# davidlougheed/strkit

Measured on NVIDIA B200. Metric: read x locus repeat counts per second, higher is better.
Workload: dtype u16x2/int32

## Files before the change

strkit_b200/csrc/api.cu:

```cuda
#include <algorithm>
#include <chrono>
#include <cmath>
#include <cstdarg>
#include <cstdio>
#include <cstdlib>
#include <cstring>
#include <mutex>
#include <new>
#include <vector>

#include "../../include/strkit_b200.h"
#include "dp_general.cuh"
#include "dp_packed.cuh"
#include "plan.cuh"
#include "dedupe.cuh"
#include "int_peak.cuh"
#include "replay.cuh"
#include "ref_path.cuh"
#include "strk_common.cuh"

static thread_local char g_err[512] = "";

static int set_err(int code, const char *fmt, ...) {
    va_list ap;
// ... 1525 lines not shown
                    const int fl = lens[3 * l], fr = lens[3 * l + 2], m = motif_len[l];
                    lists.add(strk_pk_class(fl, lens[3 * l + 1], fr, m), (int)l, m, fl, fr);
                }
                if (ctx->fallback.reserve(n) != cudaSuccess) {
                    cudaGetLastError();
                    return set_err(STRK_ERR_NOMEM, "strk_ref_counts: cannot allocate the fallback list");
                }
                const int *seg_list[STRK_PK_NBIN];
                long long seg_cnt[STRK_PK_NBIN];
                int seg_w[STRK_PK_NBIN];
                for (int k = 0; k < STRK_PK_NBIN; ++k) seg_w[k] = 2 * stride_w - 1;
                rc = lists.upload(d.lists, st, seg_list, seg_cnt);
                if (rc) return rc;
                CU(cudaMemsetAsync(ctx->d_queue + 2, 0, sizeof(unsigned int), st));
                long long n_packed = 0;
                rc = launch_pass(ctx, seg_list, seg_cnt, lists.flank, lists.mmax, seg_w, n_loci, ctx->fams.p, d.arena.p,
                                 ctx->table64.p, b_len, rowlen, st, 1, &n_packed);
                if (rc) return rc;
                CU(cudaStreamSynchronize(st));
            } else {
                rc = launch_general(ctx, true, ctx->fams.p, nullptr, n_pending, d.arena.p, ctx->table64.p, b_len, rowlen, st);
                if (rc) return rc;
            }
            CU(cudaEventRecord(ctx->ev[1], st));
            CU(cudaMemsetAsync(d.cnt.p, 0, 4 * sizeof(unsigned int), st));
            ref_replay1_kernel<<<(unsigned)((n_pending + T - 1) / T), T, 0, st>>>(
                d_ids, (int)n_pending, ctx->table64.p, ctx->fams.p, d.start.p, d.rc.p, d.ref_size.p, vcf_anchor_size, WD_MAX,
                d.wd.p, d.l_off.p, d.r_off.p, d.n_off.p, d_again, d.cnt.p);
            CU(cudaGetLastError());
            CU(cudaEventRecord(ctx->ev[2], st));
            ctx->stats[2] += 2;
            unsigned int h_cnt[4] = {0, 0, 0, 0};
            CU(cudaMemcpyAsync(h_cnt, d.cnt.p, sizeof(h_cnt), cudaMemcpyDeviceToHost, st));
            CU(cudaStreamSynchronize(st));
            {
                float t0 = 0.f, t1 = 0.f;
                CU(cudaEventElapsedTime(&t0, ctx->ev[0], ctx->ev[1]));
                CU(cudaEventElapsedTime(&t1, ctx->ev[1], ctx->ev[2]));
                acc_stats[3] += t0;
                acc_stats[4] += t1;
            }
            if (h_cnt[2])
                return set_err(STRK_ERR_SEARCH, "strk_ref_counts: locus %lld left the widest window",
                               (long long)(0x7fffffffu - h_cnt[2]));
            if (h_cnt[1]) {
                const long long l = (long long)(0x7fffffffu - h_cnt[1]);
                return set_err(STRK_ERR_SEARCH, "strk_ref_counts: locus %lld scored no size (max_iters = %d)", l,
                               rc_params[3 * l]);
            }
            n_pending = h_cnt[0];
            acc_stats[5] += (double)n_pending;
            d_ids = d_again;
            d_again = d_again == d.ids_a.p ? d.ids_b.p : d.ids_a.p;
            cur_wd = std::min(WD_MAX, cur_wd * 4);
        }
    }
    const double t_phase1 = now();
    acc_stats[2] = ctx->stats[2];
    std::vector<int> l_off(n), r_off(n), n_off(n);
    CU(cudaMemcpyAsync(l_off.data(), d.l_off.p, n * sizeof(int), cudaMemcpyDeviceToHost, st));
    CU(cudaMemcpyAsync(r_off.data(), d.r_off.p, n * sizeof(int), cudaMemcpyDeviceToHost, st));
    CU(cudaMemcpyAsync(n_off.data(), d.n_off.p, n * sizeof(int), cudaMemcpyDeviceToHost, st));

    std::vector<std::vector<int>> tiers;
    std::vector<int> tier_key;
    for (int64_t l = 0; l < n_loci; ++l) {
        size_t t = 0;
        for (; t < tiers.size(); ++t)
            if (tier_key[3 * t] == rc_params[3 * l] && tier_key[3 * t + 1] == rc_params[3 * l + 1] &&
                tier_key[3 * t + 2] == rc_params[3 * l + 2])
                break;
        if (t == tiers.size()) {
            tiers.emplace_back();
            tier_key.insert(tier_key.end(), rc_params + 3 * l, rc_params + 3 * l + 3);
        }
        tiers[t].push_back((int)l);
    }
    if (!ctx->ref_batch) ctx->ref_batch = new (std::nothrow) strk_batch();
    if (!ctx->ref_batch) return set_err(STRK_ERR_NOMEM, "out of host memory");
    strk_batch *b = ctx->ref_batch;
    std::vector<int> res;
    for (size_t t = 0; t < tiers.size(); ++t) {
        const std::vector<int> &ids = tiers[t];
        const size_t nt = ids.size();
        const cudaError_t e = batch_bind(b, (long long)nt, (long long)nt);
        if (e != cudaSuccess) {
            cudaGetLastError();
            return set_err(STRK_ERR_NOMEM, "strk_ref_counts: %s", cudaGetErrorString(e));
        }
        b->d_arena = d.arena.p;
        b->h_read_begin.resize(nt + 1);
        for (size_t q = 0; q <= nt; ++q) b->h_read_begin[q] = (long long)q;
        CU(cudaMemcpyAsync(d.ids_a.p, ids.data(), nt * sizeof(int), cudaMemcpyHostToDevice, st));
        ref_plan2_kernel<<<(unsigned)((nt + T - 1) / T), T, 0, st>>>(d.ids_a.p, (int)nt, d.seq_off.p, d.lens.p, d.start.p,
                                                                     d.motif_off.p, d.motif_len.p, d.l_off.p, d.r_off.p,
                                                                     b->d_seq_off, b->d_lens, b->d_est, b->d_motif_off,
                                                                     b->d_motif_len, b->d_read_begin);
        CU(cudaGetLastError());
        CU(cudaStreamSynchronize(st));
        rc = batch_plan(ctx, b, arena_bytes);
        if (rc) return rc;
        rc = strk_batch_run(ctx, b, tier_key[3 * t], tier_key[3 * t + 1], tier_key[3 * t + 2], STRK_KERNEL_AUTO, nullptr);
        if (rc) return rc;
        for (int k = 0; k < 8; ++k) acc_stats[k] += ctx->stats[k];
        res.resize(nt * 4);
        CU(cudaMemcpy(res.data(), b->d_out, nt * 4 * sizeof(int), cudaMemcpyDeviceToHost));
        for (size_t q = 0; q < nt; ++q) {
            const int l = ids[q];
            int32_t *o = out + 8 * (size_t)l;
            o[0] = res[4 * q], o[1] = res[4 * q + 1], o[2] = l_off[(size_t)l], o[3] = r_off[(size_t)l];
            o[4] = n_off[(size_t)l], o[5] = res[4 * q + 2];
            o[6] = lens[3 * l] - std::max(0, l_off[(size_t)l]);
            o[7] = lens[3 * l + 2] - std::max(0, r_off[(size_t)l]);
        }
    }
    for (int k = 0; k < 8; ++k) ctx->stats[k] = acc_stats[k];
    if (timing)
        fprintf(stderr, "[strk_ref_counts] %lld loci: upload + phase 1 %.2f ms, phase 2 %.2f ms (host clock); DP kernels %.2f ms, "
                "replay kernels %.2f ms (device clock), %d kernels\n", (long long)n_loci, t_phase1 - t_begin, now() - t_phase1,
                acc_stats[3], acc_stats[4], (int)acc_stats[2]);
    return STRK_OK;
}

static int ref_counts_fast(strk_ctx *ctx, const uint8_t *arena, uint64_t arena_bytes, const uint64_t *seq_off,
                           const int32_t *lens, const int32_t *start_count, const int32_t *ref_size,
                           const int32_t *rc_params, int64_t n_loci, const uint64_t *motif_off, const int32_t *motif_len,
                           int vcf_anchor_size, int32_t *out, std::vector<int> &redo, bool *taken) {
    *taken = false;
    if (!ctx->h_consts.packed_ok) return STRK_OK;
    for (int64_t l = 1; l < n_loci; ++l)
        if (rc_params[3 * l] != rc_params[0] || rc_params[3 * l + 1] != rc_params[1] || rc_params[3 * l + 2] != rc_params[2])
            return STRK_OK;
    const int max_iters = rc_params[0], range = rc_params[1], step = rc_params[2];
    if (max_iters < 0 || range < 0 || step < 0 || range > 1000 || step > 1000)
        return set_err(STRK_ERR_ARG, "strk_ref_counts: bad search parameters");
    const int wd1 = ref_first_wd(range, step);
    const int stride_w = 2 * wd1 + 1;
    int wd2 = range + step + 2;
    if (wd2 < 6) wd2 = 6;
    const int W2 = 2 * wd2 + 1;
    if (2 * stride_w > PK_WINDOW_MAX || W2 > PK_WINDOW_MAX) return STRK_OK;
    *taken = true;
    cudaStream_t st = ctx->stream;
    int rc = ref_setup(ctx, st, arena, arena_bytes, seq_off, lens, start_count, ref_size, rc_params, n_loci, motif_off,
                       motif_len);
    if (rc) return rc;
    RefBufs &d = ctx->ref;
    const size_t n = (size_t)n_loci;
    int max_n1 = 0, mb_cols = 0, mb_m = 0;
    ClassLists &lists = d.classes;
    lists.clear();
    double cells1 = 0.0;
    for (int64_t l = 0; l < n_loci; ++l) {
        const int fl = lens[3 * l], tr = lens[3 * l + 1], fr = lens[3 * l + 2], m = motif_len[l];
        const int n1 = fl + tr + fr;
        max_n1 = std::max(max_n1, n1);
        if (n1 > 32 * 16) {
            mb_cols = std::max(mb_cols, std::max(fl, fr) + m * (start_count[l] + (fl + fr) / m + 1));
            mb_m = std::max(mb_m, m);
        }
        lists.add(strk_pk_class(fl, tr, fr, m), (int)l, m, fl, fr);
        cells1 += (double)n1 * ((double)fl + fr + 2.0 * m * ((double)start_count[l] + wd1));
    }
    if (!ctx->ref_batch) ctx->ref_batch = new (std::nothrow) strk_batch();
    if (!ctx->ref_batch) return set_err(STRK_ERR_NOMEM, "out of host memory");
    strk_batch *b = ctx->ref_batch;
    const int CAP2 = 4096;
    const int WD_MAX = (STRK_MAX_WINDOW - 1) / 2;
    const int wd1b = std::min(WD_MAX, 4 * wd1), stride_w2 = 2 * wd1b + 1;
    cudaError_t e = d.out.reserve(8 * n + 8);
    if (e == cudaSuccess) e = batch_bind(b, (long long)n, (long long)n);
    if (e == cudaSuccess) e = ctx->fams.reserve(std::max(n, (size_t)CAP2));
    if (e == cudaSuccess) e = ctx->table64.reserve(std::max(n * (size_t)stride_w * 2, (size_t)CAP2 * (size_t)stride_w2 * 2));
    if (e == cudaSuccess) e = ctx->table.reserve(n * (size_t)W2);
    if (e == cudaSuccess) e = ctx->fallback.reserve(n);
    if (e != cudaSuccess) {
        cudaGetLastError();
        return set_err(STRK_ERR_NOMEM, "strk_ref_counts: %s", cudaGetErrorString(e));
    }
    b->d_arena = d.arena.p;
    const int *seg_list[STRK_PK_NBIN];
    long long seg_cnt[STRK_PK_NBIN];
    rc = lists.upload(d.lists, st, seg_list, seg_cnt);
    if (rc) return rc;
    CU(cudaMemsetAsync(d.cnt.p, 0, 8 * sizeof(unsigned int), st));
    CU(cudaMemsetAsync(ctx->d_acc, 0, 4 * sizeof(double), st));
    CU(cudaMemsetAsync(ctx->d_queue + 1, 0, 3 * sizeof(unsigned int), st));
    const int T = 128;
    const int b_len = max_n1 + 2;
    const int rowlen = max_n1 > 32 * 16 ? mb_cols + mb_m * std::max(std::max(wd1, wd2), wd1b) + 2 : 2;
    int seg_w1[STRK_PK_NBIN], seg_w2[STRK_PK_NBIN];
    for (int k = 0; k < STRK_PK_NBIN; ++k) {
        seg_w1[k] = 2 * stride_w - 1;
        seg_w2[k] = (W2 + 3) / 4 * 4;
    }
    ref_plan1_kernel<<<(unsigned)((n + T - 1) / T), T, 0, st>>>(nullptr, (int)n, d.seq_off.p, d.lens.p, d.start.p, d.wd.p,
                                                               d.motif_off.p, d.motif_len.p, stride_w, ctx->fams.p);
    CU(cudaGetLastError());
    CU(cudaEventRecord(ctx->ev[0], st));
    long long n_packed = 0;
    rc = launch_pass(ctx, seg_list, seg_cnt, lists.flank, lists.mmax, seg_w1, n_loci, ctx->fams.p, d.arena.p, ctx->table64.p,
                     b_len, rowlen, st, 1, &n_packed);
    if (rc) return rc;
    CU(cudaEventRecord(ctx->ev[1], st));
    ref_replay1_kernel<<<(unsigned)((n + T - 1) / T), T, 0, st>>>(nullptr, (int)n, ctx->table64.p, ctx->fams.p, d.start.p, d.rc.p,
                                                                 d.ref_size.p, vcf_anchor_size, WD_MAX, d.wd.p, d.l_off.p,
                                                                 d.r_off.p, d.n_off.p, d.ids_a.p, d.cnt.p);
    CU(cudaGetLastError());
    {
        ref_clamp_count_kernel<<<1, 32, 0, st>>>(d.cnt.p, (unsigned)CAP2);
        ref_plan1_kernel<<<(unsigned)((CAP2 + T - 1) / T), T, 0, st>>>(d.ids_a.p, CAP2, d.seq_off.p, d.lens.p, d.start.p, d.wd.p,
                                                                      d.motif_off.p, d.motif_len.p, stride_w2, ctx->fams.p, d.cnt.p);
        CU(cudaGetLastError());
        rc = launch_general(ctx, true, ctx->fams.p, nullptr, CAP2, d.arena.p, ctx->table64.p, b_len, rowlen, st, d.cnt.p);
        if (rc) return rc;
        ref_replay1_kernel<<<(unsigned)((CAP2 + T - 1) / T), T, 0, st>>>(d.ids_a.p, CAP2, ctx->table64.p, ctx->fams.p, d.start.p,
                                                                        d.rc.p, d.ref_size.p, vcf_anchor_size, WD_MAX, d.wd.p,
                                                                        d.l_off.p, d.r_off.p, d.n_off.p, d.ids_b.p, d.cnt.p + 4,
                                                                        d.cnt.p);
        CU(cudaGetLastError());
    }
    ref_plan2_kernel<<<(unsigned)((n + T - 1) / T), T, 0, st>>>(nullptr, (int)n, d.seq_off.p, d.lens.p, d.start.p, d.motif_off.p,
                                                               d.motif_len.p, d.l_off.p, d.r_off.p, b->d_seq_off, b->d_lens,
                                                               b->d_est, b->d_motif_off, b->d_motif_len, b->d_read_begin,
                                                               b->d_read_locus);
    CU(cudaGetLastError());
    plan_reads_kernel<<<(unsigned)((n + 255) / 256), 256, 0, st>>>(nullptr, (long long)n, b->d_seq_off, b->d_lens, b->d_est,
                                                                  b->d_read_locus, b->d_motif_off, b->d_motif_len, wd2, 0, W2,
                                                                  ctx->fams.p, ctx->d_acc + 1, nullptr);
    CU(cudaGetLastError());
    CU(cudaEventRecord(ctx->ev[2], st));
    CU(cudaMemsetAsync(ctx->d_queue + 2, 0, sizeof(unsigned int), st));
    long long n_packed2 = 0;
    rc = launch_pass(ctx, seg_list, seg_cnt, lists.flank, lists.mmax, seg_w2, n_loci, ctx->fams.p, d.arena.p, ctx->table.p, b_len,
                     rowlen, st, 0, &n_packed2);
    if (rc) return rc;
    CU(cudaEventRecord(ctx->ev[3], st));
    rc = launch_replay(ctx, b, W2, wd2, 0, nullptr, nullptr, (long long)n, max_iters, range, step, nullptr, nullptr, st);
    if (rc) return rc;
    ref_assemble_kernel<<<(unsigned)((n + T - 1) / T), T, 0, st>>>((int)n, b->d_out, b->d_status, d.lens.p, d.l_off.p, d.r_off.p,
                                                                  d.n_off.p, d.out.p);
    CU(cudaGetLastError());
    CU(cudaEventRecord(ctx->ev[4], st));
    std::vector<unsigned char> status(n);
    unsigned int h_cnt[8] = {0, 0, 0, 0, 0, 0, 0, 0};
    double acc[2] = {0, 0};
    CU(cudaMemcpyAsync(out, d.out.p, 8 * n * sizeof(int), cudaMemcpyDeviceToHost, st));
    CU(cudaMemcpyAsync(status.data(), b->d_status, n, cudaMemcpyDeviceToHost, st));
    CU(cudaMemcpyAsync(h_cnt, d.cnt.p, sizeof(h_cnt), cudaMemcpyDeviceToHost, st));
    CU(cudaMemcpyAsync(acc, ctx->d_acc, sizeof(acc), cudaMemcpyDeviceToHost, st));
    CU(cudaStreamSynchronize(st));
    if (h_cnt[1] || h_cnt[5]) {
        const long long l = (long long)(0x7fffffffu - (h_cnt[1] ? h_cnt[1] : h_cnt[5]));
        return set_err(STRK_ERR_SEARCH, "strk_ref_counts: locus %lld scored no size (max_iters = %d)", l, max_iters);
    }
    for (size_t l = 0; l < n; ++l)
        if (status[l] || out[8 * l + 4] < 0) redo.push_back((int)l);
    float t1 = 0.f, t2 = 0.f, t3 = 0.f, t4 = 0.f;
    CU(cudaEventElapsedTime(&t1, ctx->ev[0], ctx->ev[1]));
    CU(cudaEventElapsedTime(&t2, ctx->ev[1], ctx->ev[2]));
    CU(cudaEventElapsedTime(&t3, ctx->ev[2], ctx->ev[3]));
    CU(cudaEventElapsedTime(&t4, ctx->ev[3], ctx->ev[4]));
    ctx->stats[0] = cells1 + acc[1];
    ctx->stats[1] = acc[0];
    ctx->stats[2] += 7;
    ctx->stats[3] = t1 + t3;
    ctx->stats[4] = t2 + t4;
    ctx->stats[5] = 0;
    if (getenv("STRK_REF_TIMING"))
        fprintf(stderr, "[strk_ref_counts] fast path, %lld loci: DP kernels %.2f + %.2f ms, replay / second look / planning kernels "
                "%.2f + %.2f ms (device clock), %u loci took the second look, %zu left to redo\n", (long long)n_loci, t1, t3, t2, t4,
                h_cnt[0], redo.size());
    return STRK_OK;
}

extern "C" int strk_measure_int_peak(strk_ctx *ctx, double out_tiops[3]) {
    if (!ctx || !out_tiops) return set_err(STRK_ERR_ARG, "strk_measure_int_peak: null argument");
    CU(cudaSetDevice(ctx->device));
    int *d_out = (int *)(ctx->d_queue + 7);
    const int grid = ctx->n_sm * 8, threads = 256, iters = 4096;
    const double instr = (double)grid * threads * (double)iters * 64.0;
    cudaEvent_t e0 = ctx->ev[0], e1 = ctx->ev[1];
    for (int mode = 0; mode < 3; ++mode) {
        float best = 1e30f;
        for (int rep = 0; rep < 4; ++rep) {
            CU(cudaEventRecord(e0, ctx->stream));
            if (mode == 0) int_peak_kernel<0><<<grid, threads, 0, ctx->stream>>>(iters, rep + 3, d_out);
            if (mode == 1) int_peak_kernel<1><<<grid, threads, 0, ctx->stream>>>(iters, rep + 3, d_out);
            if (mode == 2) int_peak_kernel<2><<<grid, threads, 0, ctx->stream>>>(iters, rep + 3, d_out);
            CU(cudaGetLastError());
            CU(cudaEventRecord(e1, ctx->stream));
            CU(cudaEventSynchronize(e1));
            float ms = 0.f;
            CU(cudaEventElapsedTime(&ms, e0, e1));
            if (rep > 0 && ms < best) best = ms;
        }
        out_tiops[mode] = instr / ((double)best * 1e-3) / 1e12;
    }
    return STRK_OK;
}

#include "alleles_api.cuh"
#include "realign_api.cuh"
```

strkit_b200/csrc/dp_packed.cuh:

```cuda
#pragma once
#include "dp_general.cuh"
#include "strk_common.cuh"

#define PK_FLANK_MAX 160
#define PK_WINDOW_MAX 128
#ifndef PK_WARPS
#define PK_WARPS 4
#endif
#ifndef PK_WARPS_PAIRED
#define PK_WARPS_PAIRED 4
#endif
__host__ __device__ constexpr int pk_warps(int L) { return L == 16 ? PK_WARPS_PAIRED : PK_WARPS; }
#ifndef PK_PROF_IMAD
#define PK_PROF_IMAD 0
#endif
#ifndef PK_ONE_VREG
#define PK_ONE_VREG 0
#endif
#ifndef PK_MIN_CTAS
#define PK_MIN_CTAS(R) ((R) <= 10 ? 5 : ((R) <= 18 ? 4 : 3))
#endif

struct PackedDims {
    int colt_entries;
    int prof_words;
    int w_max;
};

__host__ __device__ inline int pk_quads(int R) { return (R + 1 + 3) / 4; }
__host__ __device__ inline int pk_prof_rows(int R) { return (R + 1) / 2 * 2; }
__host__ __device__ inline int pk_prof_words(int R, int m, int L = 32) { return m * pk_prof_rows(R) * L; }
__host__ __device__ inline size_t pk_scratch_words_per_unit(int R, int w_max, int L = 32) {
    return (size_t)(w_max + 1) * pk_quads(R) * L * 4;
}
__host__ __device__ inline size_t pk_code_bytes(int R, int L = 32) { return (size_t)(2 * L * R + 128 + 15) / 16 * 16; }
__host__ __device__ inline size_t pk_smem16_per_unit(int R, const PackedDims &d, int L = 32) {
    return (size_t)d.colt_entries + ((size_t)d.prof_words * 4 + 15) / 16 + pk_code_bytes(R, L) / 16;
}
__host__ __device__ inline size_t pk_smem_bytes(int R, const PackedDims &d, int L = 32) {
    return pk_smem16_per_unit(R, d, L) * 16 * pk_warps(L) * (32 / L);
}

__device__ __forceinline__ unsigned pk_prmt(unsigned a, unsigned b, unsigned sel) {
    unsigned r;
    asm("prmt.b32 %0, %1, %2, %3;" : "=r"(r) : "r"(a), "r"(b), "r"(sel));
    return r;
}

__device__ __forceinline__ unsigned pk_add(unsigned a, unsigned b, unsigned one) {
    unsigned r;
    asm("mad.lo.u32 %0, %1, %2, %3;" : "=r"(r) : "r"(a), "r"(one), "r"(b));
    return r;
}

__device__ __forceinline__ void pk_max3_inplace(unsigned &h, unsigned t, unsigned u) {
    asm("{.reg .b32 t1; \n\t"
        "max.u16x2 t1, %1, %2; \n\t"
        "max.u16x2 %0, t1, %0;}\n\t"
        : "+r"(h) : "r"(t), "r"(u));
}

template <int R>
struct PkState {
    unsigned H[R];
    unsigned selA[R];
    unsigned selB[R];
    unsigned prev_up, topv, pm;
    int poff;
    int cand_step;
    unsigned foff;
    int cand_stepB;
    unsigned boff;
    unsigned long long pol;
};

#ifndef PK_SCRATCH_POLICY
#define PK_SCRATCH_POLICY 0
#endif
__device__ __forceinline__ unsigned long long pk_l2_policy() {
    unsigned long long pol = 0ull;
#if PK_SCRATCH_POLICY & 2
    asm volatile("createpolicy.fractional.L2::evict_last.b64 %0, 1.0;" : "=l"(pol));
#endif
    return pol;
}
__device__ __forceinline__ void pk_discard_line(const void *p) {
#if PK_SCRATCH_POLICY & 1
    asm volatile("discard.global.L2 [%0], 128;" ::"l"(p) : "memory");
#endif
}
__device__ __forceinline__ void pk_st4(unsigned *p, unsigned a, unsigned b, unsigned c, unsigned d, unsigned on,
                                       unsigned long long pol) {
    (void)pol;
#if PK_SCRATCH_POLICY & 2
    asm volatile("{ .reg .pred p; setp.ne.u32 p, %5, 0; @p st.global.L2::cache_hint.v4.u32 [%0], {%1, %2, %3, %4}, %6; }" ::"l"(p),
                 "r"(a), "r"(b), "r"(c), "r"(d), "r"(on), "l"(pol)
                 : "memory");
#else
    asm volatile("{ .reg .pred p; setp.ne.u32 p, %5, 0; @p st.global.v4.u32 [%0], {%1, %2, %3, %4}; }" ::"l"(p), "r"(a),
                 "r"(b), "r"(c), "r"(d), "r"(on)
                 : "memory");
#endif
}
__device__ __forceinline__ void pk_st2(unsigned *p, unsigned a, unsigned b, unsigned on) {
    asm volatile("{ .reg .pred p; setp.ne.u32 p, %3, 0; @p st.global.v2.u32 [%0], {%1, %2}; }" ::"l"(p), "r"(a), "r"(b), "r"(on)
                 : "memory");
}
__device__ __forceinline__ void pk_st1(unsigned *p, unsigned a, unsigned on) {
    asm volatile("{ .reg .pred p; setp.ne.u32 p, %2, 0; @p st.global.u32 [%0], %1; }" ::"l"(p), "r"(a), "r"(on) : "memory");
}

template <int R, int L>
__device__ __forceinline__ void pk_capture(const PkState<R> &st, uint4 *__restrict__ dst, const unsigned on) {
    constexpr int QF = R / 4, REM = R % 4;
#pragma unroll
    for (int q = 0; q < QF; ++q)
        pk_st4((unsigned *)(dst + q * L), st.H[4 * q], st.H[4 * q + 1], st.H[4 * q + 2], st.H[4 * q + 3], on, st.pol);
    unsigned *tail = (unsigned *)(dst + QF * L);
    if (REM == 1) {
        pk_st2(tail, st.H[R - 1], st.pm, on);
    } else if (REM == 2) {
        pk_st2(tail, st.H[R - 2], st.H[R - 1], on);
        pk_st1(tail + 2, st.pm, on);
    } else if (REM == 3) {
        pk_st2(tail, st.H[R - 3], st.H[R - 2], on);
        pk_st2(tail + 2, st.H[R - 1], st.pm, on);
    } else {
        pk_st1(tail, st.pm, on);
    }
}

enum { PK_CORE_FLANK2 = 0, PK_CORE_FLANK1 = 1, PK_CORE_PROF = 2, PK_CORE_FLANK1R = 3, PK_CORE_FLANK0 = 4 };

template <int R, int L, int CORE, bool FC, bool BC>
__device__ __forceinline__ void pk_run(PkState<R> &st, int &s, const int s_end, const bool lane0, const int lane,
                                       const unsigned one, const unsigned tinc, const unsigned ginc, const uint4 *__restrict__ ctp,
                                       const unsigned *__restrict__ prof_lane, const int pstride, const int pwrap,
                                       const int m, const int last_cand_step, const int last_cand_stepB,
                                       uint4 *__restrict__ scr) {
    constexpr int QN = (R + 1 + 3) / 4;
#pragma unroll 1
    for (; s < s_end; ++s) {
        unsigned up_in = __shfl_up_sync(0xffffffffu, st.H[R - 1], 1, L);
        st.topv += tinc;
        up_in = lane0 ? st.topv : up_in;
        unsigned d = st.prev_up, u = up_in;
        st.prev_up = up_in;
        if (CORE == PK_CORE_PROF) {
            const uint2 *pp = (const uint2 *)prof_lane + st.poff;
            unsigned sc[(R + 1) / 2 * 2];
#pragma unroll
            for (int q = 0; q < (R + 1) / 2; ++q) {
                const uint2 v = pp[q * L];
                sc[2 * q] = v.x;
                sc[2 * q + 1] = v.y;
            }
            unsigned t[R];
#if PK_PROF_IMAD
            t[0] = pk_add(d, sc[0], one);
#pragma unroll
            for (int r = 1; r < R; ++r) t[r] = pk_add(st.H[r - 1], sc[r], one);
#else
            t[0] = d + sc[0];
#pragma unroll
            for (int r = 1; r < R; ++r) t[r] = st.H[r - 1] + sc[r];
#endif
#pragma unroll
            for (int r = 0; r < R; ++r) {
                pk_max3_inplace(st.H[r], t[r], u);
                u = st.H[r];
            }
            st.poff = st.poff + pstride == pwrap ? 0 : st.poff + pstride;
        } else {
            const uint4 ct = ctp[s];
            const unsigned started = s >= lane ? one : 0u;
            unsigned t[R];
#pragma unroll
            for (int r = 0; r < R; ++r) {
                const unsigned dd = r == 0 ? d : st.H[r == 0 ? 0 : r - 1];
                if (CORE == PK_CORE_FLANK0)
                    t[r] = pk_add(dd, pk_prmt(ct.x, ct.z, st.selA[r]), one);
                else if (CORE == PK_CORE_FLANK1)
                    t[r] = pk_add(pk_add(dd, pk_prmt(ct.x, ct.z, st.selA[r]), one), st.selB[r], one);
                else if (CORE == PK_CORE_FLANK1R)
                    t[r] = pk_add(st.selB[r], pk_add(dd, pk_prmt(ct.x, ct.z, st.selA[r]), one), started);
                else
                    t[r] = pk_add(pk_add(dd, pk_prmt(ct.x, ct.y, st.selA[r]), one), pk_prmt(ct.z, ct.w, st.selB[r]), one);
            }
#pragma unroll
            for (int r = 0; r < R; ++r) {
                pk_max3_inplace(st.H[r], t[r], u);
                u = st.H[r];
            }
        }
        st.pm = __viaddmax_u16x2(st.pm, ginc, st.H[R - 1]);
        if (FC) {
            const bool hit = s == st.cand_step;
            pk_capture<R, L>(st, scr + st.foff, hit ? 1u : 0u);
            const int nxt = st.cand_step + m;
            st.foff += hit ? QN * L : 0;
            st.cand_step = hit ? (nxt > last_cand_step ? 0x7fffffff : nxt) : st.cand_step;
        }
        if (BC) {
            const bool hit = s == st.cand_stepB;
            pk_capture<R, L>(st, scr + st.boff, hit ? 1u : 0u);
            const int nxt = st.cand_stepB + m;
            st.boff += hit ? QN * L : 0;
            st.cand_stepB = hit ? (nxt > last_cand_stepB ? 0x7fffffff : nxt) : st.cand_stepB;
        }
    }
}

template <int R, int L>
__global__ void __launch_bounds__(pk_warps(L) * 32, PK_MIN_CTAS(R) * PK_WARPS / pk_warps(L))
dp_packed_kernel(const FamDesc *__restrict__ fams, const int *__restrict__ list, int n_list,
                 const unsigned char *__restrict__ arena, const ScoreConsts *__restrict__ consts,
                 int *__restrict__ table, PackedDims dims, uint4 *__restrict__ scratch,
                 int *__restrict__ fallback_list, unsigned int *__restrict__ fallback_count, int ref_mode,
                 unsigned int *__restrict__ work_counter) {
    static_assert(R >= 2 && (L == 32 || L == 16), "rows per lane / lanes per read out of range");
    constexpr int HALVES = 32 / L;
    constexpr int SK = L - 1;
    constexpr int N = L * R;
    constexpr int QN = (R + 1 + 3) / 4;
    constexpr int RH = (R + 1) / 2;
    extern __shared__ uint4 smem_raw[];
    __shared__ SmemConsts sc;
    __shared__ unsigned long long t8f[STRK_NSYM_], t8b[STRK_NSYM_];
    __shared__ unsigned rowinfo[STRK_SMAT_ROWS + 1];
    for (int k = threadIdx.x; k < 256; k += blockDim.x) sc.lut[k] = consts->lut[k];
    for (int k = threadIdx.x; k < STRK_SMAT_ROWS * STRK_NSYM_; k += blockDim.x) sc.smat[k] = consts->smat[k];
    for (int k = threadIdx.x; k < STRK_NSYM_; k += blockDim.x) {
        t8f[k] = consts->t8f[k];
        t8b[k] = consts->t8b[k];
    }
    for (int k = threadIdx.x; k <= STRK_SMAT_ROWS; k += blockDim.x) rowinfo[k] = consts->rowinfo[k];
    __syncthreads();

    const int wlane = threadIdx.x & 31;
    const int lane = wlane & (L - 1);
    const int half = wlane / L;
    const unsigned hmask = L == 32 ? 0xffffffffu : (0xffffu << (16 * half));
    const int warp = threadIdx.x >> 5;
    const int unit = warp * HALVES + half;
    const int unit_global = (blockIdx.x * pk_warps(L) + warp) * HALVES + half;
    const int total_units = gridDim.x * pk_warps(L) * HALVES;
    const int g = consts->gap;
    const int flags = ref_mode ? 0 : consts->end_flags;
    const bool one_table_ok = consts->one_table_ok != 0;
#if PK_ONE_VREG
    const unsigned one = consts->one_v[wlane];
#else
    const unsigned one = consts->one_v[0];
#endif
    const bool s1_beg = flags & 1, s1_end = flags & 2, s2_beg = flags & 4, s2_end = flags & 8;
    const bool lane0 = lane == 0;
    auto all_unit = [&](bool pred) -> bool { return (__ballot_sync(0xffffffffu, pred) & hmask) == hmask; };

    uint4 *colT = smem_raw + (size_t)unit * pk_smem16_per_unit(R, dims, L);
    unsigned *prof = (unsigned *)(colT + dims.colt_entries);
    unsigned char *rowF = (unsigned char *)(prof + (dims.prof_words + 3) / 4 * 4);
    unsigned char *rowB = rowF + N;
    unsigned char *mcodes = rowB + N;
    uint4 *scr = scratch + (size_t)unit_global * (size_t)(dims.w_max + 1) * QN * L;
    const unsigned tinc = (s2_beg ? (unsigned)g : 0u) | ((s2_end ? (unsigned)g : 0u) << 16);
    const unsigned ginc = (unsigned)g | ((unsigned)g << 16);
    const int g2 = 2 * g;

    (void)total_units;
    for (;;) {
        unsigned int base = 0u;
        if (wlane == 0) base = atomicAdd(work_counter, (unsigned int)HALVES);
        base = __shfl_sync(0xffffffffu, base, 0);
        if (base >= (unsigned int)n_list) break;
        const int fam_idx_raw = (int)base + half;
        const bool have = fam_idx_raw < n_list;
        if (!__any_sync(0xffffffffu, have)) break;
        const int fam_id = list[have ? fam_idx_raw : n_list - 1];
        const FamDesc f = fams[fam_id];
        const int n1 = f.n_fl + f.n_tr + f.n_fr;
        const int off = N - n1;
        const int m = f.m;
        const unsigned char *db = arena + f.db_off;
        const unsigned char *motif = arena + f.motif_off;

        int b0 = (m * f.n_hi + f.n_fl - f.n_fr + m) / (2 * m);
        b0 = b0 < 0 ? 0 : (b0 > f.n_lo ? f.n_lo : b0);
        if (ref_mode) b0 = 0;
        const int a_lo = f.n_lo - b0, a_hi = f.n_hi - b0;
        const int nW = a_hi - a_lo + 1;
        const int nWB = ref_mode ? nW : 1;
        if (ref_mode) b0 = f.n_hi;
        const int colsF = f.n_fl + m * a_hi, colsB = f.n_fr + m * b0;
        const int ncols = colsF > colsB ? colsF : colsB;
        const int Lmax = __reduce_max_sync(0xffffffffu, f.n_fl > f.n_fr ? f.n_fl : f.n_fr);

        bool ok = off >= 1 && f.n_fl >= 1 && f.n_fr >= 1 && Lmax <= PK_FLANK_MAX && Lmax + 2 * SK + 2 <= dims.colt_entries &&
                  pk_prof_words(R, m, L) <= dims.prof_words && m <= 128 && nW + nWB <= dims.w_max + 1 &&
                  (g * (N + ncols + 40) + 2 * N + 1024) < (ref_mode ? 32000 : 65535);
        ok = __all_sync(0xffffffffu, ok);
        if (!ok) {
            if (lane0 && have) fallback_list[atomicAdd(fallback_count, 1u)] = fam_id;
            continue;
        }
        __syncwarp();

        bool motif_acgt = true;
        for (int d = lane; d < n1; d += L) {
            const unsigned char c = sc.lut[db[d]];
            rowF[d + off] = c;
            rowB[N - 1 - d] = c;
        }
        for (int I = lane; I < off; I += L) rowF[I] = rowB[I] = (unsigned char)STRK_PAD_PEN;
        for (int k = lane; k < m; k += L) {
            const unsigned char c = sc.lut[motif[k]];
            mcodes[k] = c;
            motif_acgt = motif_acgt && c < 4;
        }
        motif_acgt = all_unit(motif_acgt);
        __syncwarp();

        const unsigned inv_m = (1048576u + (unsigned)m - 1u) / (unsigned)m;
        auto mod_m = [&](int x) -> int { return x - (int)(((unsigned)x * inv_m) >> 20) * m; };

        bool acgt = true;
        for (int e = lane; e <= Lmax + 2 * SK; e += L) {
            const int j = e - SK;
            uint4 v = make_uint4(0u, 0u, 0u, 0u);
            if (j >= 1) {
                const int sf = j <= f.n_fl ? rowF[off + j - 1] : mcodes[mod_m(j - f.n_fl - 1)];
                const int sb = j <= f.n_fr ? rowF[N - j] : mcodes[m - 1 - mod_m(j - f.n_fr - 1)];
                acgt = acgt && sf < 4 && sb < 4;
                const unsigned long long a = t8f[sf], b = t8b[sb];
                v = make_uint4((unsigned)a, (unsigned)(a >> 32), (unsigned)b, (unsigned)(b >> 32));
            }
            colT[e] = v;
        }
        const bool cols_acgt = all_unit(acgt);

        PkState<R> st;
        const unsigned char *myF = rowF + lane * R, *myB = rowB + lane * R;
        unsigned flags_or = 0u;
#pragma unroll
        for (int r = 0; r < R; ++r) {
            const unsigned wf = rowinfo[myF[r]], wb = rowinfo[myB[r]];
            flags_or |= wf | wb;
            st.selA[r] = (wf & 0xfu) | ((wb & 0xf0u) << 4) | 0x8080u;
            st.selB[r] = ((wf >> 16) & 0xffu) | (wb & 0xff0000u);
        }
        const bool rows_ok = !(flags_or & 0x800u);
        const bool rows_plain = !(flags_or & 0x1000u);
        if (!__all_sync(0xffffffffu, rows_ok)) {
            if (lane0 && have) fallback_list[atomicAdd(fallback_count, 1u)] = fam_id;
            continue;
        }
        const bool no_addend = __all_sync(0xffffffffu, rows_plain);
        const bool plain_unit = all_unit(rows_plain);
        const bool one_table = __all_sync(0xffffffffu, (one_table_ok && cols_acgt) || plain_unit);
        if (one_table_ok && motif_acgt) {
            for (int k = 0; k < m; ++k) {
                const unsigned tf = (unsigned)t8f[mcodes[mod_m(k + Lmax - f.n_fl)]];
                const unsigned tb = (unsigned)t8b[mcodes[m - 1 - mod_m(k + Lmax - f.n_fr)]];
#pragma unroll
                for (int r = 0; r < R; ++r)
                    prof[((k * RH + (r >> 1)) * L + lane) * 2 + (r & 1)] = pk_prmt(tf, tb, st.selA[r]) + st.selB[r];
            }
        } else {
            for (int k = 0; k < m; ++k) {
                const int sf = mcodes[mod_m(k + Lmax - f.n_fl)];
                const int sb = mcodes[m - 1 - mod_m(k + Lmax - f.n_fr)];
#pragma unroll
                for (int r = 0; r < R; ++r) {
                    const int vf = sc.smat[myF[r] * STRK_NSYM_ + sf] + g2;
                    const int vb = sc.smat[myB[r] * STRK_NSYM_ + sb] + g2;
                    prof[((k * RH + (r >> 1)) * L + lane) * 2 + (r & 1)] = (unsigned)vf | ((unsigned)vb << 16);
                }
            }
        }
        if (!one_table) {
#pragma unroll
            for (int r = 0; r < R; ++r) {
                st.selA[r] = ((rowinfo[myF[r]] >> 8) & 7u) | 0x8880u;
                st.selB[r] = (((rowinfo[myB[r]] >> 8) & 7u) << 8) | 0x8088u;
            }
        }

#pragma unroll
        for (int r = 0; r < R; ++r) {
            const int I = lane * R + r + 1, i = I - off;
            int vf = g * off, vb = g * off;
            if (i >= 1) {
                vf = (s1_beg ? 0 : -g * i) + g * I;
                vb = (s1_end ? (i == n1 ? -g : 0) : -g * i) + g * I;
            }
            st.H[r] = (unsigned)vf | ((unsigned)vb << 16);
        }
        {
            const int I = lane * R, i = I - off;
            int vf = g * off, vb = g * off;
            if (i >= 1) {
                vf = (s1_beg ? 0 : -g * i) + g * I;
                vb = (s1_end ? 0 : -g * i) + g * I;
            }
            st.prev_up = (unsigned)vf | ((unsigned)vb << 16);
        }
        st.topv = (unsigned)(g * off) | ((unsigned)(g * off) << 16);
        st.pm = 0u;
        st.poff = 0;
        st.foff = (unsigned)lane;
        st.boff = (unsigned)(nW * (QN * L) + lane);
        st.pol = pk_l2_policy();

        const int first_cand = f.n_fl + m * a_lo;
        const int first_candB = colsB - m * (nWB - 1);
        const int nsteps = __reduce_max_sync(0xffffffffu, ncols + SK);
        const int s_star = Lmax + SK < nsteps ? Lmax + SK : nsteps;
        const int fc_begin = __reduce_min_sync(0xffffffffu, first_cand - 1);
        const int bc_begin = __reduce_min_sync(0xffffffffu, first_candB - 1);
        const int bc_end = __reduce_max_sync(0xffffffffu, colsB + SK);
        st.cand_step = first_cand + lane - 1;
        st.cand_stepB = first_candB + lane - 1;
        const int last_cand_step = colsF + lane - 1;
        const int last_cand_stepB = colsB + lane - 1;
        const uint4 *ctp = colT + (SK + 1) - lane;
        const unsigned *prof_lane = prof + 2 * lane;
        const int pstride = RH * L, pwrap = m * RH * L;
        __syncwarp();

#define PK_RUN(CORE, FC, BC, END)                                                                          \
    pk_run<R, L, CORE, FC, BC>(st, s, END, lane0, lane, one, tinc, ginc, ctp, prof_lane, pstride, pwrap, m,     \
                               last_cand_step, last_cand_stepB, scr)

        int s = 0;
        {
            const int e0 = s_star < SK ? s_star : SK;
            const bool ramp_caps = fc_begin < e0 || bc_begin < e0;
            if (no_addend) {
                if (ramp_caps)
                    PK_RUN(PK_CORE_FLANK0, true, true, e0);
                else
                    PK_RUN(PK_CORE_FLANK0, false, false, e0);
            } else if (one_table) {
                if (ramp_caps)
                    PK_RUN(PK_CORE_FLANK1R, true, true, e0);
                else
                    PK_RUN(PK_CORE_FLANK1R, false, false, e0);
            } else {
                if (ramp_caps)
                    PK_RUN(PK_CORE_FLANK2, true, true, e0);
                else
                    PK_RUN(PK_CORE_FLANK2, false, false, e0);
            }
            st.pm = 0u;
            while (s < s_star) {
                const bool fc = s >= fc_begin, bc = s >= bc_begin && s < bc_end;
                int e = s_star;
                if (fc_begin > s && fc_begin < e) e = fc_begin;
                if (bc_begin > s && bc_begin < e) e = bc_begin;
                if (bc_end > s && bc_end < e) e = bc_end;
                if (no_addend) {
                    if (fc || bc)
                        PK_RUN(PK_CORE_FLANK0, true, true, e);
                    else
                        PK_RUN(PK_CORE_FLANK0, false, false, e);
                } else if (one_table) {
                    if (fc || bc)
                        PK_RUN(PK_CORE_FLANK1, true, true, e);
                    else
                        PK_RUN(PK_CORE_FLANK1, false, false, e);
                } else {
                    if (fc || bc)
                        PK_RUN(PK_CORE_FLANK2, true, true, e);
                    else
                        PK_RUN(PK_CORE_FLANK2, false, false, e);
                }
            }
        }
        if (s < nsteps) {
            st.poff = mod_m(s - lane - Lmax) * pstride;
            while (s < nsteps) {
                const bool fc = s >= fc_begin, bc = s >= bc_begin && s < bc_end;
                int e = nsteps;
                if (fc_begin > s && fc_begin < e) e = fc_begin;
                if (bc_begin > s && bc_begin < e) e = bc_begin;
                if (bc_end > s && bc_end < e) e = bc_end;
                if (fc) {
                    if (bc)
                        PK_RUN(PK_CORE_PROF, true, true, e);
                    else
                        PK_RUN(PK_CORE_PROF, true, false, e);
                } else {
                    if (bc)
                        PK_RUN(PK_CORE_PROF, false, true, e);
                    else
                        PK_RUN(PK_CORE_PROF, false, false, e);
                }
            }
        }
#undef PK_RUN

        __syncwarp();
        if (ref_mode) {
            long long *out64 = (long long *)table + 2 * f.out_off;
            for (int w2 = 0; w2 < 2 * nW; ++w2) {
                const int dir = w2 >= nW, w = dir ? w2 - nW : w2;
                const int p = (dir ? f.n_fr : f.n_fl) + m * (f.n_lo + w);
                unsigned key = 0u;
#pragma unroll
                for (int q = 0; q < QN; ++q) {
                    const uint4 v = scr[(unsigned)((w2 * QN + q) * L + lane)];
                    const unsigned wv[4] = {v.x, v.y, v.z, v.w};
#pragma unroll
                    for (int j = 0; j < 4; ++j) {
                        const int r = 4 * q + j;
                        if (r < R) {
                            const int I = lane * R + r + 1, i = I - off;
                            const int h = (int)(dir ? wv[j] >> 16 : wv[j] & 0xffffu);
                            const unsigned k = ((unsigned)(h - g * (I + p) + 32768) << 16) | (unsigned)(0xffff - i);
                            if (i >= 1) key = max(key, k);
                        }
                    }
                }
                key = __reduce_max_sync(hmask, key);
                if (lane0 && have) {
                    const int score = (int)(key >> 16) - 32768, row = 0xffff - (int)(key & 0xffffu);
                    out64[w2] = ((long long)score << 32) | (long long)(unsigned)(0x7fffffff - row);
                }
            }
            __syncwarp();
            for (int ln = lane; ln < 2 * nW * QN * L / 8; ln += L) pk_discard_line(scr + ln * 8);
            __syncwarp();
            continue;
        }
        const unsigned *scw = (const unsigned *)scr;
        const unsigned bbase = (unsigned)nW * (QN * L * 4);
        unsigned Bv[R];
        {
            int ib1 = N + off - (lane * R + 1) - 1;
            int lb = ib1 / R, rb = ib1 - lb * R;
#pragma unroll
            for (int r = 0; r < R; ++r) {
                unsigned v = 0u;
                if (lane * R + r + 1 >= off) v = scw[bbase + (unsigned)(((rb >> 2) * L + lb) * 4 + (rb & 3))] >> 16;
                Bv[r] = v;
                if (--rb < 0) rb = R - 1, --lb;
            }
        }
        const int bextra = (int)(scw[bbase + (unsigned)(((R >> 2) * L + (L - 1)) * 4 + (R & 3))] >> 16);
        constexpr int WB = 4;
        for (int g0 = 0; g0 < nW; g0 += L) {
            const int gend = g0 + L < nW ? g0 + L : nW;
            unsigned my_v = 0u, my_flast = 0u;
            for (int w0 = g0; w0 < gend; w0 += WB) {
                uint4 q4[WB][QN];
#pragma unroll
                for (int b = 0; b < WB; ++b) {
                    const int ww = w0 + b < gend ? w0 + b : gend - 1;
#pragma unroll
                    for (int q = 0; q < QN; ++q) q4[b][q] = scr[(unsigned)((ww * QN + q) * L + lane)];
                }
#pragma unroll
                for (int b = 0; b < WB; ++b) {
                    const int ww = w0 + b;
                    if (ww >= gend) break;
                    unsigned acc = 0u;
#pragma unroll
                    for (int q = 0; q < QN; ++q) {
                        const uint4 v = q4[b][q];
                        if (4 * q + 0 < R) acc = __viaddmax_u16x2(v.x, Bv[(4 * q + 0) % R], acc);
                        if (4 * q + 1 < R) acc = __viaddmax_u16x2(v.y, Bv[(4 * q + 1) % R], acc);
                        if (4 * q + 2 < R) acc = __viaddmax_u16x2(v.z, Bv[(4 * q + 2) % R], acc);
                        if (4 * q + 3 < R) acc = __viaddmax_u16x2(v.w, Bv[(4 * q + 3) % R], acc);
                    }
                    const unsigned v = __reduce_max_sync(hmask, acc & 0xffffu);
                    const unsigned pmw = (&q4[b][R >> 2].x)[R & 3];
                    const unsigned flast = __shfl_sync(hmask, pmw, L - 1, L) & 0xffffu;
                    if (lane == ww - g0) my_v = v, my_flast = flast;
                }
            }
            if (g0 + lane < gend && have) {
                const int p = f.n_fl + m * (a_lo + g0 + lane);
                int best = (int)my_v - g * (N + off + p + colsB);
                if (s2_end) best = max(best, (int)my_flast - g * (N + p));
                if (s2_beg) {
                    const int border = s1_end ? -g : -g * n1;
                    best = max(best, max(bextra - g * (N + colsB), border));
                }
                table[f.out_off + g0 + lane] = best;
            }
        }
        __syncwarp();
        for (int ln = lane; ln < (nW + 1) * QN * L / 8; ln += L) pk_discard_line(scr + ln * 8);
        __syncwarp();
    }
}
```

Measured before the change: 70.80 million.

## Prefetch work items, restructure profile build and candidate reductions, add phase timers

The work-queue atomic is now issued one iteration ahead, so the next family index is fetched while the current one is being processed. The motif profile fill uses incremental indices instead of a modulo per k. The ref-mode and normal candidate scans are restructured: fixed-size batches with a scalar tail replace the clamped batch loop, and the per-row key math is precomputed into registers and combined with prmt. The last-column value is read directly from scratch instead of through a shuffle per candidate. Optional clock64 phase timers are added behind a compile flag, off by default.

```diff
diff --git a/strkit_b200/csrc/api.cu b/strkit_b200/csrc/api.cu
--- a/strkit_b200/csrc/api.cu
+++ b/strkit_b200/csrc/api.cu
@@ -1851,3 +1851,17 @@
 
 #include "alleles_api.cuh"
 #include "realign_api.cuh"
+
+#if PK_PHASE_TIMERS
+extern "C" int strk_pk_phase_timers(int device, unsigned long long *out, int reset) {
+    if (!out) return set_err(STRK_ERR_ARG, "strk_pk_phase_timers: null argument");
+    CU(cudaSetDevice(device));
+    CU(cudaDeviceSynchronize());
+    CU(cudaMemcpyFromSymbol(out, pk_phase_clk, sizeof(pk_phase_clk)));
+    if (reset) {
+        static const unsigned long long zero[2 * 2 * 17 * 4] = {0ull};
+        CU(cudaMemcpyToSymbol(pk_phase_clk, zero, sizeof(pk_phase_clk)));
+    }
+    return STRK_OK;
+}
+#endif
diff --git a/strkit_b200/csrc/dp_packed.cuh b/strkit_b200/csrc/dp_packed.cuh
--- a/strkit_b200/csrc/dp_packed.cuh
+++ b/strkit_b200/csrc/dp_packed.cuh
@@ -19,6 +19,13 @@
 #endif
 #ifndef PK_MIN_CTAS
 #define PK_MIN_CTAS(R) ((R) <= 10 ? 5 : ((R) <= 18 ? 4 : 3))
+#endif
+
+#ifndef PK_PHASE_TIMERS
+#define PK_PHASE_TIMERS 0
+#endif
+#if PK_PHASE_TIMERS
+__device__ unsigned long long pk_phase_clk[2][2][17][4];
 #endif
 
 struct PackedDims {
@@ -211,6 +218,19 @@
     }
 }
 
+template <int R, int QN>
+__device__ __forceinline__ unsigned pk_cand_max(const uint4 (&c)[QN], const unsigned (&Bv)[R]) {
+    unsigned acc = 0u;
+#pragma unroll
+    for (int q = 0; q < QN; ++q) {
+        if (4 * q + 0 < R) acc = __viaddmax_u16x2(c[q].x, Bv[(4 * q + 0) % R], acc);
+        if (4 * q + 1 < R) acc = __viaddmax_u16x2(c[q].y, Bv[(4 * q + 1) % R], acc);
+        if (4 * q + 2 < R) acc = __viaddmax_u16x2(c[q].z, Bv[(4 * q + 2) % R], acc);
+        if (4 * q + 3 < R) acc = __viaddmax_u16x2(c[q].w, Bv[(4 * q + 3) % R], acc);
+    }
+    return acc & 0xffffu;
+}
+
 template <int R, int L>
 __global__ void __launch_bounds__(pk_warps(L) * 32, PK_MIN_CTAS(R) * PK_WARPS / pk_warps(L))
 dp_packed_kernel(const FamDesc *__restrict__ fams, const int *__restrict__ list, int n_list,
@@ -224,6 +244,8 @@
     constexpr int N = L * R;
     constexpr int QN = (R + 1 + 3) / 4;
     constexpr int RH = (R + 1) / 2;
+    constexpr int WB = 4;
+    constexpr int WBR = 2;
     extern __shared__ uint4 smem_raw[];
     __shared__ SmemConsts sc;
     __shared__ unsigned long long t8f[STRK_NSYM_], t8b[STRK_NSYM_];
@@ -267,12 +289,30 @@
     const unsigned ginc = (unsigned)g | ((unsigned)g << 16);
     const int g2 = 2 * g;
 
-    (void)total_units;
-    for (;;) {
-        unsigned int base = 0u;
-        if (wlane == 0) base = atomicAdd(work_counter, (unsigned int)HALVES);
-        base = __shfl_sync(0xffffffffu, base, 0);
+#if PK_PHASE_TIMERS
+    unsigned long long clk_acc[4] = {0ull, 0ull, 0ull, 0ull}, clk_t = clock64();
+#define PK_CLK(P)                                      \
+    do {                                               \
+        const unsigned long long t_ = clock64();       \
+        clk_acc[P] += t_ - clk_t;                      \
+        clk_t = t_;                                    \
+    } while (0)
+#else
+#define PK_CLK(P) \
+    do {          \
+    } while (0)
+#endif
+    unsigned int next = 0u;
+    auto pop = [&] {
+        if (wlane == 0) next = atomicAdd(work_counter, (unsigned int)HALVES);
+    };
+    pop();
+    bool ahead = false;
+    for (;; ahead ? (void)0 : pop()) {
+        const unsigned int base = __shfl_sync(0xffffffffu, next, 0);
         if (base >= (unsigned int)n_list) break;
+        ahead = base + 2u * (unsigned int)total_units < (unsigned int)n_list;
+        if (ahead) pop();
         const int fam_idx_raw = (int)base + half;
         const bool have = fam_idx_raw < n_list;
         if (!__any_sync(0xffffffffu, have)) break;
@@ -357,23 +397,28 @@
         const bool no_addend = __all_sync(0xffffffffu, rows_plain);
         const bool plain_unit = all_unit(rows_plain);
         const bool one_table = __all_sync(0xffffffffu, (one_table_ok && cols_acgt) || plain_unit);
-        if (one_table_ok && motif_acgt) {
-            for (int k = 0; k < m; ++k) {
-                const unsigned tf = (unsigned)t8f[mcodes[mod_m(k + Lmax - f.n_fl)]];
-                const unsigned tb = (unsigned)t8b[mcodes[m - 1 - mod_m(k + Lmax - f.n_fr)]];
-#pragma unroll
-                for (int r = 0; r < R; ++r)
-                    prof[((k * RH + (r >> 1)) * L + lane) * 2 + (r & 1)] = pk_prmt(tf, tb, st.selA[r]) + st.selB[r];
-            }
-        } else {
-            for (int k = 0; k < m; ++k) {
-                const int sf = mcodes[mod_m(k + Lmax - f.n_fl)];
-                const int sb = mcodes[m - 1 - mod_m(k + Lmax - f.n_fr)];
-#pragma unroll
-                for (int r = 0; r < R; ++r) {
-                    const int vf = sc.smat[myF[r] * STRK_NSYM_ + sf] + g2;
-                    const int vb = sc.smat[myB[r] * STRK_NSYM_ + sb] + g2;
-                    prof[((k * RH + (r >> 1)) * L + lane) * 2 + (r & 1)] = (unsigned)vf | ((unsigned)vb << 16);
+        {
+            int jf = mod_m(Lmax - f.n_fl), jb = m - 1 - mod_m(Lmax - f.n_fr);
+            unsigned *pc = prof + 2 * lane;
+            if (one_table_ok && motif_acgt) {
+                for (int k = 0; k < m; ++k, pc += 2 * RH * L) {
+                    const unsigned tf = (unsigned)t8f[mcodes[jf]], tb = (unsigned)t8b[mcodes[jb]];
+#pragma unroll
+                    for (int r = 0; r < R; ++r) pc[(r >> 1) * 2 * L + (r & 1)] = pk_prmt(tf, tb, st.selA[r]) + st.selB[r];
+                    jf = jf + 1 == m ? 0 : jf + 1;
+                    jb = jb == 0 ? m - 1 : jb - 1;
+                }
+            } else {
+                for (int k = 0; k < m; ++k, pc += 2 * RH * L) {
+                    const int sf = mcodes[jf], sb = mcodes[jb];
+#pragma unroll
+                    for (int r = 0; r < R; ++r) {
+                        const int vf = sc.smat[myF[r] * STRK_NSYM_ + sf] + g2;
+                        const int vb = sc.smat[myB[r] * STRK_NSYM_ + sb] + g2;
+                        pc[(r >> 1) * 2 * L + (r & 1)] = (unsigned)vf | ((unsigned)vb << 16);
+                    }
+                    jf = jf + 1 == m ? 0 : jf + 1;
+                    jb = jb == 0 ? m - 1 : jb - 1;
                 }
             }
         }
@@ -431,6 +476,7 @@
     pk_run<R, L, CORE, FC, BC>(st, s, END, lane0, lane, one, tinc, ginc, ctp, prof_lane, pstride, pwrap, m,     \
                                last_cand_step, last_cand_stepB, scr)
 
+        PK_CLK(0);
         int s = 0;
         {
             const int e0 = s_star < SK ? s_star : SK;
@@ -500,36 +546,70 @@
 #undef PK_RUN
 
         __syncwarp();
+        PK_CLK(1);
+#if PK_PHASE_TIMERS
+        clk_acc[3] += 1ull;
+#endif
         if (ref_mode) {
             long long *out64 = (long long *)table + 2 * f.out_off;
-            for (int w2 = 0; w2 < 2 * nW; ++w2) {
-                const int dir = w2 >= nW, w = dir ? w2 - nW : w2;
-                const int p = (dir ? f.n_fr : f.n_fl) + m * (f.n_lo + w);
-                unsigned key = 0u;
-#pragma unroll
-                for (int q = 0; q < QN; ++q) {
-                    const uint4 v = scr[(unsigned)((w2 * QN + q) * L + lane)];
-                    const unsigned wv[4] = {v.x, v.y, v.z, v.w};
-#pragma unroll
-                    for (int j = 0; j < 4; ++j) {
-                        const int r = 4 * q + j;
-                        if (r < R) {
-                            const int I = lane * R + r + 1, i = I - off;
-                            const int h = (int)(dir ? wv[j] >> 16 : wv[j] & 0xffffu);
-                            const unsigned k = ((unsigned)(h - g * (I + p) + 32768) << 16) | (unsigned)(0xffff - i);
-                            if (i >= 1) key = max(key, k);
+            unsigned rc[R], rk[R], rsel[R];
+#pragma unroll
+            for (int r = 0; r < R; ++r) {
+                const int I = lane * R + r + 1, i = I - off;
+                rc[r] = (unsigned)(32768 - g * I);
+                rk[r] = i >= 1 ? (unsigned)(0xffff - i) : 0u;
+                rsel[r] = i >= 1 ? 0x5410u : 0u;
+            }
+            const uint4 *col = scr + lane;
+            for (int dir = 0; dir < 2; ++dir) {
+                if (dir) {
+#pragma unroll
+                    for (int r = 0; r < R; ++r) {
+                        rc[r] <<= 16;
+                        rsel[r] = rsel[r] ? 0x7610u : 0u;
+                    }
+                }
+                const int p0 = (dir ? f.n_fr : f.n_fl) + m * f.n_lo;
+                auto column = [&](const uint4(&c)[QN], int w) {
+                    const unsigned gp = (unsigned)(-g * (p0 + m * w)), np = dir ? gp << 16 : gp;
+                    unsigned key = 0u;
+#pragma unroll
+                    for (int q = 0; q < QN; ++q) {
+                        const unsigned wv[4] = {c[q].x, c[q].y, c[q].z, c[q].w};
+#pragma unroll
+                        for (int j = 0; j < 4; ++j) {
+                            const int r = 4 * q + j;
+                            if (r < R) key = max(key, pk_prmt(rk[r], wv[j] + rc[r] + np, rsel[r]));
                         }
                     }
-                }
-                key = __reduce_max_sync(hmask, key);
-                if (lane0 && have) {
-                    const int score = (int)(key >> 16) - 32768, row = 0xffff - (int)(key & 0xffffu);
-                    out64[w2] = ((long long)score << 32) | (long long)(unsigned)(0x7fffffff - row);
+                    key = __reduce_max_sync(hmask, key);
+                    if (lane0 && have) {
+                        const int score = (int)(key >> 16) - 32768, row = 0xffff - (int)(key & 0xffffu);
+                        out64[dir * nW + w] = ((long long)score << 32) | (long long)(unsigned)(0x7fffffff - row);
+                    }
+                };
+                int w = 0;
+                for (; w + WBR <= nW; w += WBR, col += WBR * QN * L) {
+                    uint4 q4[WBR][QN];
+#pragma unroll
+                    for (int b = 0; b < WBR; ++b)
+#pragma unroll
+                        for (int q = 0; q < QN; ++q) q4[b][q] = col[(b * QN + q) * L];
+#pragma unroll
+                    for (int b = 0; b < WBR; ++b) column(q4[b], w + b);
+                }
+#pragma unroll 1
+                for (; w < nW; ++w, col += QN * L) {
+                    uint4 q1[QN];
+#pragma unroll
+                    for (int q = 0; q < QN; ++q) q1[q] = col[q * L];
+                    column(q1, w);
                 }
             }
             __syncwarp();
             for (int ln = lane; ln < 2 * nW * QN * L / 8; ln += L) pk_discard_line(scr + ln * 8);
             __syncwarp();
+            PK_CLK(2);
             continue;
         }
         const unsigned *scw = (const unsigned *)scr;
@@ -547,50 +627,58 @@
             }
         }
         const int bextra = (int)(scw[bbase + (unsigned)(((R >> 2) * L + (L - 1)) * 4 + (R & 3))] >> 16);
-        constexpr int WB = 4;
+        constexpr int CW = QN * L;
         for (int g0 = 0; g0 < nW; g0 += L) {
-            const int gend = g0 + L < nW ? g0 + L : nW;
-            unsigned my_v = 0u, my_flast = 0u;
-            for (int w0 = g0; w0 < gend; w0 += WB) {
+            const int gn = nW - g0 < L ? nW - g0 : L;
+            const uint4 *col = scr + (size_t)g0 * CW + lane;
+            unsigned my_v = 0u;
+            int k = 0;
+            for (; k + WB <= gn; k += WB, col += WB * CW) {
                 uint4 q4[WB][QN];
 #pragma unroll
+                for (int b = 0; b < WB; ++b)
+#pragma unroll
+                    for (int q = 0; q < QN; ++q) q4[b][q] = col[b * CW + q * L];
+                const int lk = lane - k;
+#pragma unroll
                 for (int b = 0; b < WB; ++b) {
-                    const int ww = w0 + b < gend ? w0 + b : gend - 1;
-#pragma unroll
-                    for (int q = 0; q < QN; ++q) q4[b][q] = scr[(unsigned)((ww * QN + q) * L + lane)];
-                }
-#pragma unroll
-                for (int b = 0; b < WB; ++b) {
-                    const int ww = w0 + b;
-                    if (ww >= gend) break;
-                    unsigned acc = 0u;
-#pragma unroll
-                    for (int q = 0; q < QN; ++q) {
-                        const uint4 v = q4[b][q];
-                        if (4 * q + 0 < R) acc = __viaddmax_u16x2(v.x, Bv[(4 * q + 0) % R], acc);
-                        if (4 * q + 1 < R) acc = __viaddmax_u16x2(v.y, Bv[(4 * q + 1) % R], acc);
-                        if (4 * q + 2 < R) acc = __viaddmax_u16x2(v.z, Bv[(4 * q + 2) % R], acc);
-                        if (4 * q + 3 < R) acc = __viaddmax_u16x2(v.w, Bv[(4 * q + 3) % R], acc);
-                    }
-                    const unsigned v = __reduce_max_sync(hmask, acc & 0xffffu);
-                    const unsigned pmw = (&q4[b][R >> 2].x)[R & 3];
-                    const unsigned flast = __shfl_sync(hmask, pmw, L - 1, L) & 0xffffu;
-                    if (lane == ww - g0) my_v = v, my_flast = flast;
-                }
-            }
-            if (g0 + lane < gend && have) {
-                const int p = f.n_fl + m * (a_lo + g0 + lane);
+                    const unsigned v = __reduce_max_sync(hmask, pk_cand_max<R, QN>(q4[b], Bv));
+                    my_v = lk == b ? v : my_v;
+                }
+            }
+#pragma unroll 1
+            for (; k < gn; ++k, col += CW) {
+                uint4 q1[QN];
+#pragma unroll
+                for (int q = 0; q < QN; ++q) q1[q] = col[q * L];
+                const unsigned v = __reduce_max_sync(hmask, pk_cand_max<R, QN>(q1, Bv));
+                my_v = lane == k ? v : my_v;
+            }
+            if (lane < gn && have) {
+                const int w = g0 + lane;
+                const int p = f.n_fl + m * (a_lo + w);
                 int best = (int)my_v - g * (N + off + p + colsB);
-                if (s2_end) best = max(best, (int)my_flast - g * (N + p));
+                if (s2_end) {
+                    const unsigned flast = scw[(unsigned)(((w * QN + (R >> 2)) * L + (L - 1)) * 4 + (R & 3))] & 0xffffu;
+                    best = max(best, (int)flast - g * (N + p));
+                }
                 if (s2_beg) {
                     const int border = s1_end ? -g : -g * n1;
                     best = max(best, max(bextra - g * (N + colsB), border));
                 }
-                table[f.out_off + g0 + lane] = best;
+                table[f.out_off + w] = best;
             }
         }
         __syncwarp();
         for (int ln = lane; ln < (nW + 1) * QN * L / 8; ln += L) pk_discard_line(scr + ln * 8);
         __syncwarp();
+        PK_CLK(2);
     }
-}
+#if PK_PHASE_TIMERS
+    if (wlane == 0) {
+        unsigned long long *acc = pk_phase_clk[ref_mode ? 1 : 0][L == 16 ? 1 : 0][R];
+        for (int k = 0; k < 4; ++k) atomicAdd(acc + k, clk_acc[k]);
+    }
+#endif
+#undef PK_CLK
+}
```

Result: faster. 73.73 million, median of 6 (+4.1%).
